# wangrui2025/GDKVM

Hardware: AMD Instinct MI355X
Metric: frames/sec (GDKVM forward + argmax mask), EchoNet 112x112x32 clips (higher is better)
Workload: dtype bf16; 1 GPU; BASELINE.json configs[1]: EchoNet-Dynamic 112x112x32 bf16 inference, batch=16 per GPU; clips_per_gpu=16, frames_per_clip=32, image=112x112, heads=1, key_dim=64, rule=delta_sequential, world_size=1, ranks_seen=1

## Files before the change

gdkvm_amd/csrc/conv3x3_tile.hip:

```cpp
#include <atomic>
#include "gdkvm_device.hpp"

namespace {

constexpr int CT_CK = 64;
constexpr int CT_PIX = 160;
constexpr int CT_SLOTS = CT_PIX / 16;
constexpr int CT_MAXMT = 13;
constexpr int CT_VARIANT_128 = 4, CT_VARIANT_64 = 3;

struct ConvTileArgs {
    const bf16_t* x; const bf16_t* w; const float* bias; const bf16_t* res; bf16_t* y;
    const bf16_t* x2; int C1;
    int N, H, W, C, K;
    int fpt, th, tiles_y, ntiles;
    int bw, bh, band_px, npieces;
    int relu;
    float inv_band, inv_bw, inv_tw, inv_w;
    int perm;
};
struct ConvUpArgs : ConvTileArgs {
    int hl, wl, nlr;
    int stage_px, nstage;
    int stage_off;
    int nrp;
    float inv_slr, inv_wl, inv_ncp, inv_nrp;
};

__host__ __device__ __forceinline__ int ct_channel(int kt, int j, int perm)
{
    return perm ? 32 * (kt >> 1) + 8 * (j >> 2) + 4 * (kt & 1) + (j & 3) : 16 * kt + j;
}

template <int NWN, int NTW, bool PK, int NWV = 8, int MAXMT = CT_MAXMT, bool UP = false>
__global__ __launch_bounds__(64 * NWV, (NWV == 4 ? 2 : 1)) void conv3x3_tile_kernel(std::conditional_t<UP, ConvUpArgs, ConvTileArgs> a)
{
    constexpr int MW = NWV / NWN, MTW = (MAXMT + MW - 1) / MW;
    extern __shared__ __attribute__((aligned(16))) unsigned char ct_band[];
    const int tid = threadIdx.x, lane = tid & 63, li = lane & 15, g = lane >> 4;
    const int w = __builtin_amdgcn_readfirstlane(tid >> 6), wn = w % NWN, wm = w / NWN;
    const int H = a.H, W = a.W, C = a.C, K = a.K, BW = a.bw;
    const int band_bytes = a.npieces * 1024, nchunk = C / CT_CK;
    const int tpix = a.fpt * a.th * W;
    const int co0 = blockIdx.y * (16 * NTW * NWN) + 16 * NTW * wn;

    f32x4 bias4[NTW];
#pragma unroll
    for (int nt = 0; nt < NTW; ++nt) {
        const int kt = min(co0 / 16 + nt, K / 16 - 1);
        const float* bp = a.bias + ct_channel(kt, 4 * g, a.perm);
        asm volatile("global_load_dwordx4 %0, %1, off" : "=&v"(bias4[nt]) : "v"(bp) : "memory");
    }

    constexpr int PP = NWV == 8 ? 7 : 8;
    const int cs1 = a.C1, cs2 = a.x2 ? C - a.C1 : C;
    unsigned g_off1[PP], g_off2[PP];
#pragma unroll
    for (int u = 0; u < PP; ++u) {
        const int j = w + NWV * u, d = 64 * j + lane, pix = d / CT_SLOTS, c = d - CT_SLOTS * pix;
        const int f = idx_div(pix, a.inv_band), r = pix - f * (a.bh * BW), by = idx_div(r, a.inv_bw), bx = r - by * BW;
        const int sp = (f * H + by - 1) * W + bx - 1;
        const bool live = j < a.npieces && c < 8 && pix < a.band_px && bx >= 1 && bx <= W && (a.tiles_y > 1 || (by >= 1 && by <= a.th));
        g_off1[u] = live ? (unsigned)(sp * cs1 * 2 + c * 16) : RSRC_DEAD;
        g_off2[u] = live ? (unsigned)(sp * cs2 * 2 + c * 16) : RSRC_DEAD;
        if constexpr (UP) {
            const int spx = d >> 3, c8 = d & 7;
            const int sf = idx_div(spx, a.inv_slr), sr = spx - sf * (a.nlr * a.wl), lr = idx_div(sr, a.inv_wl), lx = sr - lr * a.wl;
            g_off1[u] = j < a.nstage && spx < a.stage_px ? (unsigned)((((sf * a.hl + lr) * a.wl + lx) * cs1 + c8 * 8) * 2) : RSRC_DEAD;
        }
    }
    const unsigned lds0 = (unsigned)reinterpret_cast<uintptr_t>(ct_band);
    const int nlive = max(0, (a.npieces - w + NWV - 1) / NWV);
    int nlive_up = 0, stage_off = 0;
    if constexpr (UP) { nlive_up = max(0, (a.nstage - w + NWV - 1) / NWV); stage_off = a.stage_off; }
    struct Geo { int px0, npx, row0, r0, lr0, nfr; };
    auto geo_of = [&](int tile) __attribute__((always_inline)) {
        const int ty = tile % a.tiles_y, fg = tile / a.tiles_y;
        Geo q;
        q.px0 = fg * a.fpt * H * W;
        q.npx = min(a.fpt, a.N - fg * a.fpt) * H * W;
        q.row0 = ty * a.th * W;
        q.r0 = q.lr0 = q.nfr = 0;
        if constexpr (UP) {
            q.r0 = ty * a.th; q.lr0 = max((q.r0 - 2) >> 1, 0); q.nfr = min(a.fpt, a.N - fg * a.fpt);
        }
        return q;
    };
    auto fetch = [&](const Geo q, int chunk, int buf) __attribute__((always_inline)) {
        const bool second = a.x2 != nullptr && chunk * CT_CK >= a.C1;
        const int cs = second ? cs2 : cs1;
        const bool up = UP && !second;
        const bf16_t* base = (second ? a.x2 : a.x) + (long long)(up ? q.px0 >> 2 : q.px0) * cs;
        const __amdgpu_buffer_rsrc_t rsrc = make_rsrc(base, (up ? q.npx >> 2 : q.npx) * cs * 2);
        unsigned ts = (unsigned)((q.row0 * cs + chunk * CT_CK - (second ? a.C1 : 0)) * 2);
        unsigned dst0 = lds0 + buf * band_bytes + 1024 * w;
        int nl = nlive;
        if constexpr (UP) {
            ts = up ? (unsigned)((q.lr0 * (W >> 1) * cs + chunk * CT_CK) * 2) : ts;
            dst0 = up ? lds0 + stage_off + 1024 * w : dst0;
            nl = up ? nlive_up : nlive;
        }
#pragma unroll
        for (int u = 0; u < PP; ++u) {
            const unsigned dst = u < nl ? dst0 + 1024 * NWV * u : lds0 + 2 * band_bytes;
            unsigned go;
            if constexpr (UP) go = g_off1[u] ^ ((g_off1[u] ^ g_off2[u]) & (second ? ~0u : 0u));
            else go = second ? g_off2[u] : g_off1[u];
            __builtin_amdgcn_raw_ptr_buffer_load_lds(rsrc, lds_dma_dst(dst), 16, (int)(go + ts), 0, 0, 0);
        }
    };

    int tile = blockIdx.x;
    Geo cur = geo_of(min(tile, a.ntiles - 1));
    if (tile < a.ntiles) fetch(cur, 0, 0);

    unsigned pbase[MTW];
#pragma unroll
    for (int m = 0; m < MTW; ++m) {
        const int p = min(16 * (wm + MW * m) + li, tpix - 1);
        const int f = idx_div(p, a.inv_tw), r = p - f * (a.th * W), py = idx_div(r, a.inv_w), px = r - py * W;
        pbase[m] = (unsigned)(((f * a.bh + py) * BW + px) * CT_PIX + g * 16);
    }
    const bf16_t* wrow[NTW];
#pragma unroll
    for (int nt = 0; nt < NTW; ++nt) {
        const int kt = min(co0 / 16 + nt, K / 16 - 1);
        if constexpr (PK) wrow[nt] = a.w + (size_t)kt * (9 * C * 16) + lane * 8;
        else wrow[nt] = a.w + (size_t)ct_channel(kt, li, a.perm) * 9 * C + 8 * g;
    }

    const int nks = nchunk * 18;
    static_assert(NTW == 1 || NTW == 2, "wwait names the fragments of one or two output tiles");
    struct WF { bf16x8 f[NTW]; };
    auto wload = [&](WF& o, int ks) __attribute__((always_inline)) {
        ks = ks >= nks ? ks - nks : ks;
        size_t off;
        if constexpr (PK) off = (size_t)ks * 512;
        else {
            const int chunk = ks / 18, r = ks - 18 * chunk, tap = r >> 1, kh = r & 1;
            off = (size_t)tap * C + chunk * CT_CK + 32 * kh;
        }
#pragma unroll
        for (int nt = 0; nt < NTW; ++nt) asm volatile("global_load_dwordx4 %0, %1, off" : "=&v"(o.f[nt]) : "v"(wrow[nt] + off) : "memory");
    };
    auto wwait = [&](WF& o, auto nc) __attribute__((always_inline)) {
        constexpr int N = decltype(nc)::value;
        if constexpr (NTW == 1) asm volatile("s_waitcnt vmcnt(%1)" : "+v"(o.f[0]) : "n"(N) : "memory");
        else asm volatile("s_waitcnt vmcnt(%2)" : "+v"(o.f[0]), "+v"(o.f[1]) : "n"(N) : "memory");
    };
    int gc = 0;
    constexpr int WD = 3, KU = 6;
    WF wr[WD];
#pragma unroll
    for (int j = 0; j < WD; ++j) wload(wr[j], j);
    for (; tile < a.ntiles; tile += gridDim.x) {
        const Geo nxt = geo_of(min(tile + (int)gridDim.x, a.ntiles - 1));
        f32x4 acc[MTW][NTW];
#pragma unroll
        for (int m = 0; m < MTW; ++m)
#pragma unroll
            for (int nt = 0; nt < NTW; ++nt) acc[m][nt] = f32x4{0.f, 0.f, 0.f, 0.f};
        for (int chunk = 0; chunk < nchunk; ++chunk, ++gc) {
            const int buf = gc & 1;
            asm volatile("s_waitcnt vmcnt(%0) lgkmcnt(0)" ::"n"(WD * NTW) : "memory");
            asm volatile("s_barrier" ::: "memory");
            if constexpr (UP) if (chunk * CT_CK < a.C1) {
                const unsigned stg = lds0 + stage_off;
                unsigned char* const bandw = ct_band + buf * band_bytes;
                const int hl = H >> 1, wl = W >> 1, ncp = wl + 1, ip0 = (cur.r0 - 2) >> 1;
                const int nitems = a.fpt * a.nrp * ncp * 8;
#pragma unroll 1
                for (int i = tid; i < nitems; i += 64 * NWV) {
                    const int c8 = i & 7, t = i >> 3;
                    const int t2 = idx_div(t, a.inv_ncp), jp = t - t2 * ncp - 1, f = idx_div(t2, a.inv_nrp), ip = ip0 + t2 - f * a.nrp;
                    const int y0 = 2 * ip + 1, x0o = 2 * jp + 1;
                    const int by0 = y0 - cur.r0 + 1;
                    const bool vy[2] = {y0 >= 0 && y0 < H, y0 + 1 >= 0 && y0 + 1 < H}, vx[2] = {x0o >= 0, x0o + 1 < W};
                    u32x4 o[2][2] = {};
                    if ((vy[0] || vy[1]) && f < cur.nfr) {
                        const int ra = max(ip, 0) - cur.lr0, rb = min(ip + 1, hl - 1) - cur.lr0;
                        const int xa_ = max(jp, 0), xb_ = min(jp + 1, wl - 1);
                        const unsigned s0 = stg + (f * a.nlr + ra) * wl * 128 + c8 * 16, s1 = stg + (f * a.nlr + rb) * wl * 128 + c8 * 16;
                        u32x4 t00, t01, t10, t11;
                        asm volatile("ds_read_b128 %0, %1" : "=&v"(t00) : "v"(s0 + xa_ * 128) : "memory");
                        asm volatile("ds_read_b128 %0, %1" : "=&v"(t01) : "v"(s0 + xb_ * 128) : "memory");
                        asm volatile("ds_read_b128 %0, %1" : "=&v"(t10) : "v"(s1 + xa_ * 128) : "memory");
                        asm volatile("ds_read_b128 %0, %1" : "=&v"(t11) : "v"(s1 + xb_ * 128) : "memory");
                        asm volatile("s_waitcnt lgkmcnt(0)" : "+v"(t00), "+v"(t01), "+v"(t10), "+v"(t11) :: "memory");
                        const float ly[2] = {0.25f, y0 + 1 == 0 ? 0.f : 0.75f}, hy[2] = {0.75f, 1.f - ly[1]};
                        bilerp2x_bf16x8(t00, t01, t10, t11, hy, ly, o);
                    }
#pragma unroll
                    for (int ey = 0; ey < 2; ++ey) {
                        if (by0 + ey < 0 || by0 + ey >= a.bh) continue;
                        const bool rowin = vy[ey] && f < cur.nfr;
#pragma unroll
                        for (int e = 0; e < 2; ++e) {
                            const u32x4 z = {0u, 0u, 0u, 0u};
                            *reinterpret_cast<u32x4*>(bandw + ((f * a.bh + by0 + ey) * BW + x0o + 1 + e) * CT_PIX + c8 * 16) = rowin && vx[e] ? o[ey][e] : z;
                        }
                    }
                }
                asm volatile("s_waitcnt lgkmcnt(0)" ::: "memory");
                asm volatile("s_barrier" ::: "memory");
            }
            {
                const bool more = chunk + 1 < nchunk;
                Geo q;
                q.px0 = more ? cur.px0 : nxt.px0; q.npx = more ? cur.npx : nxt.npx; q.row0 = more ? cur.row0 : nxt.row0;
                q.r0 = q.lr0 = q.nfr = 0;
                if constexpr (UP) q.lr0 = more ? cur.lr0 : nxt.lr0;
                fetch(q, more ? chunk + 1 : 0, buf ^ 1);
            }
            const unsigned char* band = ct_band + buf * band_bytes;
            auto load_x = [&](bf16x8 (&xb)[MTW], int r) __attribute__((always_inline)) {
                r = min(r, 17);
                const int tap = r >> 1, kh = r & 1, dy = tap / 3, dx = tap - 3 * dy;
                const unsigned off = (unsigned)((dy * BW + dx) * CT_PIX + kh * 64);
#pragma unroll
                for (int m = 0; m < MTW; ++m) {
                    xb[m] = *reinterpret_cast<const bf16x8*>(band + pbase[m] + off);
                }
            };
            auto mfmas = [&](const bf16x8 (&xb)[MTW], const WF& wfr) __attribute__((always_inline)) {
#pragma unroll
                for (int m = 0; m < MTW; ++m)
#pragma unroll
                    for (int nt = 0; nt < NTW; ++nt) {
                        acc[m][nt] = __builtin_amdgcn_mfma_f32_16x16x32_bf16(wfr.f[nt], xb[m], acc[m][nt], 0, 0, 0);
                    }
            };
            const int ksb = chunk * 18;
            bf16x8 xa[MTW], xb[MTW];
            load_x(xa, 0);
            auto trip = [&](int r0, auto firstc) __attribute__((always_inline)) {
                constexpr bool FIRST = decltype(firstc)::value;
                static_for<0, KU>([&](auto jc) {
                    constexpr int j = decltype(jc)::value;
                    wwait(wr[j % WD], std::integral_constant<int, (WD - 1) * NTW + (FIRST && j < WD ? PP : 0)>{});
                    if constexpr (j % 2 == 0) { load_x(xb, r0 + j + 1); mfmas(xa, wr[j % WD]); }
                    else { load_x(xa, r0 + j + 1); mfmas(xb, wr[j % WD]); }
                    wload(wr[j % WD], ksb + r0 + j + WD);
                    __builtin_amdgcn_sched_barrier(0);
                });
            };
            trip(0, std::true_type{});
#pragma unroll 1
            for (int r0 = KU; r0 < 18; r0 += KU) trip(r0, std::false_type{});
        }
        {
            const int ty = tile % a.tiles_y, fg = tile / a.tiles_y;
            const float lo = a.relu ? 0.f : -INFINITY;
            if (NTW == 2 && a.perm) {
                if (co0 < K) {
                    unsigned o[MTW];
#pragma unroll
                    for (int m = 0; m < MTW; ++m) {
                        const int p = 16 * (wm + MW * m) + li;
                        const int pc = min(p, tpix - 1);
                        const int f = idx_div(pc, a.inv_tw), r = pc - f * (a.th * W), py = idx_div(r, a.inv_w), px = r - py * W;
                        const int n = fg * a.fpt + f, yy = ty * a.th + py;
                        o[m] = p < tpix && n < a.N && yy < H ? (unsigned)(((n * H + yy) * W + px) * K + co0 + 8 * g) : ~0u;
                    }
                    bf16_t* const yout = a.y;
                    const bf16_t* const resp = a.res;
                    const unsigned ofallback = (unsigned)(co0 + 8 * g);
                    auto finish = [&](auto resc) __attribute__((always_inline)) {
                        constexpr bool RES = decltype(resc)::value;
                        static_for<0, (MTW + 3) / 4>([&](auto bc) {
                            constexpr int M0 = 4 * decltype(bc)::value, M1 = M0 + 4 < MTW ? M0 + 4 : MTW;
                            u32x4 rr[4] = {};
                            if constexpr (RES) {
#pragma unroll
                                for (int m = M0; m < M1; ++m)
                                {
                                    const bf16_t* const rp = resp + (o[m] != ~0u ? o[m] : ofallback);
                                    asm volatile("global_load_dwordx4 %0, %1, off" : "=&v"(rr[m - M0]) : "v"(rp) : "memory");
                                }
                                asm volatile("s_waitcnt vmcnt(0)" : "+v"(rr[0]), "+v"(rr[1]), "+v"(rr[2]), "+v"(rr[3]) :: "memory");
                            }
#pragma unroll
                            for (int m = M0; m < M1; ++m) {
                                f32x2 v[4];
#pragma unroll
                                for (int q = 0; q < 4; ++q)
                                    v[q] = f32x2{acc[m][q >> 1][2 * (q & 1)], acc[m][q >> 1][2 * (q & 1) + 1]} + f32x2{bias4[q >> 1][2 * (q & 1)], bias4[q >> 1][2 * (q & 1) + 1]};
                                if constexpr (RES) {
#pragma unroll
                                    for (int q = 0; q < 4; ++q) v[q] += unpack_bf16x2(rr[m - M0][q]);
                                }
                                u32x4 ow;
#pragma unroll
                                for (int q = 0; q < 4; ++q) {
                                    v[q] = __builtin_elementwise_max(v[q], f32x2{lo, lo});
                                    ow[q] = pack_bf16x2(v[q][0], v[q][1]);
                                }
                                bf16_t* const yp = yout + o[m];
                                if (o[m] != ~0u) asm volatile("global_store_dwordx4 %0, %1, off\n\ts_nop 1" :: "v"(yp), "v"(ow) : "memory");
                            }
                        });
                    };
                    if (a.res) finish(std::true_type{}); else finish(std::false_type{});
                }
            } else {
#pragma unroll
                for (int m = 0; m < MTW; ++m) {
                    const int p = 16 * (wm + MW * m) + li;
                    if (p >= tpix) continue;
                    const int f = idx_div(p, a.inv_tw), r = p - f * (a.th * W), py = idx_div(r, a.inv_w), px = r - py * W;
                    const int n = fg * a.fpt + f, yy = ty * a.th + py;
                    if (n >= a.N || yy >= H) continue;
                    const size_t opix = (((size_t)n * H + yy) * W + px) * K;
#pragma unroll
                    for (int nt = 0; nt < NTW; ++nt) {
                        if (co0 + 16 * nt >= K) continue;
                        const size_t o = opix + ct_channel(co0 / 16 + nt, 4 * g, a.perm);
                        f32x4 v = acc[m][nt] + bias4[nt];
                        if (a.res) v += unpack_bf16x4(*reinterpret_cast<const uint2*>(a.res + o));
                        v = __builtin_elementwise_max(v, f32x4{lo, lo, lo, lo});
                        *reinterpret_cast<uint2*>(a.y + o) = pack_bf16x4(v);
                    }
                }
            }
        }
        cur = nxt;
    }
    asm volatile("s_waitcnt vmcnt(0)" ::: "memory");
}

__global__ __launch_bounds__(256) void conv3x3_pack_kernel(const uint4* w, uint4* packed, int K, int C)
{
    const int nks = C / CT_CK * 18;
    const size_t total = (size_t)(K / 16) * nks * 64;
    for (size_t i = (size_t)blockIdx.x * 256 + threadIdx.x; i < total; i += (size_t)gridDim.x * 256) {
        const int lane = (int)(i & 63), li = lane & 15, g = lane >> 4;
        const size_t f = i >> 6;
        const int ks = (int)(f % nks), kt = (int)(f / nks);
        const int chunk = ks / 18, r = ks - 18 * chunk, tap = r >> 1, kh = r & 1;
        packed[i] = w[(((size_t)ct_channel(kt, li, K % 32 == 0) * 9 + tap) * C + chunk * CT_CK + 32 * kh + 8 * g) / 8];
    }
}

__global__ __launch_bounds__(256) void conv3x3_pack_dgrad_kernel(const bf16_t* w, uint4* packed, int K, int C)
{
    const int nks = K / CT_CK * 18;
    const size_t total = (size_t)(C / 16) * nks * 64;
    for (size_t i = (size_t)blockIdx.x * 256 + threadIdx.x; i < total; i += (size_t)gridDim.x * 256) {
        const int lane = (int)(i & 63), li = lane & 15, g = lane >> 4;
        const size_t f = i >> 6;
        const int ks = (int)(f % nks), ct = (int)(f / nks);
        const int chunk = ks / 18, r = ks - 18 * chunk, tap = r >> 1, kh = r & 1;
        const int c = ct_channel(ct, li, C % 32 == 0), ftap = 8 - tap;
        const bf16_t* src = w + ((size_t)(chunk * CT_CK + 32 * kh + 8 * g) * 9 + ftap) * C + c;
        unsigned short e[8];
#pragma unroll
        for (int j = 0; j < 8; ++j) e[j] = src[(size_t)j * 9 * C];
        packed[i] = make_uint4(e[0] | (unsigned)e[1] << 16, e[2] | (unsigned)e[3] << 16, e[4] | (unsigned)e[5] << 16, e[6] | (unsigned)e[7] << 16);
    }
}

}

struct PackTrainLayer { const float* w; uint4* fwd; uint4* dgrad; int K, C; long long sK, sC, sR, sS; };
struct PackTrainArgs { PackTrainLayer l[GDKVM_PACK_MAX_LAYERS]; };

namespace {
__global__ __launch_bounds__(256) void conv3x3_pack_train_kernel(PackTrainArgs a)
{
    const PackTrainLayer L = a.l[blockIdx.y];
    if (!L.w) return;
    const int K = L.K, C = L.C;
    const size_t nf = (size_t)(K / 16) * (C / CT_CK * 18) * 64, nd = (size_t)(C / 16) * (K / CT_CK * 18) * 64;
    for (size_t i = (size_t)blockIdx.x * 256 + threadIdx.x; i < nf + nd; i += (size_t)gridDim.x * 256) {
        const bool fwd = i < nf;
        const size_t ii = fwd ? i : i - nf;
        const int lane = (int)(ii & 63), li = lane & 15, g = lane >> 4;
        const size_t f = ii >> 6;
        float e[8];
        if (fwd) {
            const int nks = C / CT_CK * 18, ks = (int)(f % nks), kt = (int)(f / nks);
            const int chunk = ks / 18, r = ks - 18 * chunk, tap = r >> 1, kh = r & 1;
            const float* src = L.w + (long long)ct_channel(kt, li, K % 32 == 0) * L.sK + (long long)(tap / 3) * L.sR + (long long)(tap % 3) * L.sS
                               + (long long)(chunk * CT_CK + 32 * kh + 8 * g) * L.sC;
#pragma unroll
            for (int j = 0; j < 8; ++j) e[j] = src[(long long)j * L.sC];
        } else {
            const int nks = K / CT_CK * 18, ks = (int)(f % nks), ct = (int)(f / nks);
            const int chunk = ks / 18, r = ks - 18 * chunk, tap = r >> 1, kh = r & 1, ftap = 8 - tap;
            const float* src = L.w + (long long)ct_channel(ct, li, C % 32 == 0) * L.sC + (long long)(ftap / 3) * L.sR + (long long)(ftap % 3) * L.sS
                               + (long long)(chunk * CT_CK + 32 * kh + 8 * g) * L.sK;
#pragma unroll
            for (int j = 0; j < 8; ++j) e[j] = src[(long long)j * L.sK];
        }
        const uint4 o = pack_bf16x8(e);
        (fwd ? L.fwd : L.dgrad)[ii] = o;
    }
}
}

extern "C" int gdkvm_conv3x3_pack_weights_train(int nlayers, const void* const* w, void* const* packed_fwd, void* const* packed_dgrad,
                                                const int* K, const int* C, const long long* strides, void* stream)
{
    if (nlayers < 0 || nlayers > GDKVM_PACK_MAX_LAYERS) return gdkvm_fail(GDKVM_ERR_SHAPE, "conv3x3_pack_weights_train: %d layers (at most %d per call)", nlayers, GDKVM_PACK_MAX_LAYERS);
    if (nlayers == 0) return GDKVM_OK;
    if (!w || !packed_fwd || !packed_dgrad || !K || !C || !strides) return gdkvm_fail(GDKVM_ERR_ARG, "conv3x3_pack_weights_train: null pointer");
    PackTrainArgs a{};
    for (int i = 0; i < nlayers; ++i) {
        if (K[i] <= 0 || C[i] <= 0 || K[i] % CT_CK || C[i] % CT_CK)
            return gdkvm_fail(GDKVM_ERR_SHAPE, "conv3x3_pack_weights_train: layer %d K=%d C=%d (multiples of 64)", i, K[i], C[i]);
        if (!w[i] || !packed_fwd[i] || !packed_dgrad[i] || !gdkvm_aligned16(packed_fwd[i]) || !gdkvm_aligned16(packed_dgrad[i]))
            return gdkvm_fail(GDKVM_ERR_ARG, "conv3x3_pack_weights_train: layer %d: null or unaligned pointer", i);
        a.l[i] = PackTrainLayer{static_cast<const float*>(w[i]), static_cast<uint4*>(packed_fwd[i]), static_cast<uint4*>(packed_dgrad[i]), K[i], C[i],
                                strides[4 * i], strides[4 * i + 1], strides[4 * i + 2], strides[4 * i + 3]};
    }
    if (int rc = gdkvm_check_device()) return rc;
    hipLaunchKernelGGL(conv3x3_pack_train_kernel, dim3(48, (unsigned)nlayers), dim3(256), 0, static_cast<hipStream_t>(stream), a);
    GDKVM_LAUNCH_CHECK("conv3x3_pack_train_kernel");
    return GDKVM_OK;
}

extern "C" int gdkvm_conv3x3_pack_weights_dgrad(const void* w, void* packed, int K, int C, int io_dtype, void* stream)
{
    if (io_dtype != GDKVM_BF16) return gdkvm_fail(GDKVM_ERR_DTYPE, "conv3x3_pack_weights_dgrad: only bf16 is implemented");
    if (K <= 0 || C <= 0 || K % CT_CK || C % 16) return gdkvm_fail(GDKVM_ERR_SHAPE, "conv3x3_pack_weights_dgrad: K=%d C=%d (K a multiple of 64, C of 16)", K, C);
    if (!w || !packed || !gdkvm_aligned16(w) || !gdkvm_aligned16(packed)) return gdkvm_fail(GDKVM_ERR_ARG, "conv3x3_pack_weights_dgrad: null or unaligned pointer");
    if (int rc = gdkvm_check_device()) return rc;
    const size_t total = (size_t)(C / 16) * (K / CT_CK * 18) * 64;
    hipLaunchKernelGGL(conv3x3_pack_dgrad_kernel, dim3((unsigned)((total + 255) / 256)), dim3(256), 0, static_cast<hipStream_t>(stream),
                       static_cast<const bf16_t*>(w), static_cast<uint4*>(packed), K, C);
    GDKVM_LAUNCH_CHECK("conv3x3_pack_dgrad_kernel");
    return GDKVM_OK;
}

extern "C" int gdkvm_conv3x3_pack_weights(const void* w, void* packed, int K, int C, int io_dtype, void* stream)
{
    if (io_dtype != GDKVM_BF16) return gdkvm_fail(GDKVM_ERR_DTYPE, "conv3x3_pack_weights: only bf16 is implemented");
    if (K <= 0 || C <= 0 || K % 16 || C % CT_CK) return gdkvm_fail(GDKVM_ERR_SHAPE, "conv3x3_pack_weights: K=%d C=%d (K a multiple of 16, C of 64)", K, C);
    if (!w || !packed || !gdkvm_aligned16(w) || !gdkvm_aligned16(packed)) return gdkvm_fail(GDKVM_ERR_ARG, "conv3x3_pack_weights: null or unaligned pointer");
    if (int rc = gdkvm_check_device()) return rc;
    const size_t total = (size_t)(K / 16) * (C / CT_CK * 18) * 64;
    hipLaunchKernelGGL(conv3x3_pack_kernel, dim3((unsigned)((total + 255) / 256)), dim3(256), 0, static_cast<hipStream_t>(stream),
                       static_cast<const uint4*>(w), static_cast<uint4*>(packed), K, C);
    GDKVM_LAUNCH_CHECK("conv3x3_pack_kernel");
    return GDKVM_OK;
}

namespace {
template <int NWN, int NTW, int NWV = 8, int MAXMT = CT_MAXMT>
void launch_tile(bool packed, dim3 grid, size_t lds, hipStream_t st, const ConvTileArgs& a)
{
    if (packed) hipLaunchKernelGGL((conv3x3_tile_kernel<NWN, NTW, true, NWV, MAXMT>), grid, dim3(64 * NWV), lds, st, a);
    else hipLaunchKernelGGL((conv3x3_tile_kernel<NWN, NTW, false, NWV, MAXMT>), grid, dim3(64 * NWV), lds, st, a);
}
template <int NWN, int NTW, int NWV = 8, int MAXMT = CT_MAXMT>
bool setattr_tile()
{
    return hipFuncSetAttribute(reinterpret_cast<const void*>(conv3x3_tile_kernel<NWN, NTW, true, NWV, MAXMT>), hipFuncAttributeMaxDynamicSharedMemorySize, 113 * 1024) == hipSuccess
        && hipFuncSetAttribute(reinterpret_cast<const void*>(conv3x3_tile_kernel<NWN, NTW, false, NWV, MAXMT>), hipFuncAttributeMaxDynamicSharedMemorySize, 113 * 1024) == hipSuccess;
}
constexpr size_t CT_UP_LDS = 80 * 1024;
template <int NWN, int NTW>
bool setattr_up()
{
    return hipFuncSetAttribute(reinterpret_cast<const void*>(conv3x3_tile_kernel<NWN, NTW, true, 4, 7, true>), hipFuncAttributeMaxDynamicSharedMemorySize, (int)CT_UP_LDS) == hipSuccess;
}

bool tile_geometry(ConvTileArgs& a, int maxpix, int maxpieces)
{
    const int N = a.N, H = a.H, W = a.W;
    if (H * W <= maxpix) { a.th = H; a.fpt = maxpix / (H * W); a.tiles_y = 1; if (a.fpt > N) a.fpt = N; }
    else { a.fpt = 1; a.th = maxpix / W; if (a.th < 1) return false; a.tiles_y = (H + a.th - 1) / a.th; }
    a.bw = W + 2; a.bh = a.th + 2;
    auto pieces = [&]() { a.band_px = a.fpt * a.bh * a.bw; return (a.band_px * CT_SLOTS + 63) / 64; };
    while (pieces() > maxpieces && a.fpt > 1) --a.fpt;
    while (pieces() > maxpieces && a.th > 1) { --a.th; a.bh = a.th + 2; a.tiles_y = (H + a.th - 1) / a.th; }
    a.npieces = pieces();
    if (a.npieces > maxpieces) return false;
    a.inv_band = 1.0f / (float)(a.bh * a.bw); a.inv_bw = 1.0f / (float)a.bw;
    a.inv_tw = 1.0f / (float)(a.th * W); a.inv_w = 1.0f / (float)W;
    const long long groups = (N + a.fpt - 1) / a.fpt;
    const long long ntiles = groups * a.tiles_y;
    if (ntiles <= 0 || ntiles > 0x7fffffffLL) return false;
    a.ntiles = (int)ntiles;
    return true;
}
}

int gdkvm_conv3x3_upcat_launch(const void* lo, const void* x2, int C1, const void* w, const float* bias, const void* residual, void* y,
                               int N, int C, int H, int W, int K, int relu, hipStream_t st)
{
    if (C % CT_CK || K % 16 || W > 64 || W < 2 || H < 2 || (H | W) & 1 || N < 1 || !x2 || C1 <= 0 || C1 >= C || C1 % CT_CK) return 1;
    ConvUpArgs a;
    a.x2 = static_cast<const bf16_t*>(x2); a.C1 = C1;
    a.x = static_cast<const bf16_t*>(lo); a.w = static_cast<const bf16_t*>(w); a.bias = bias;
    a.res = static_cast<const bf16_t*>(residual); a.y = static_cast<bf16_t*>(y);
    a.N = N; a.H = H; a.W = W; a.C = C; a.K = K; a.relu = relu;
    if (!tile_geometry(a, 16 * 7, 32)) return 1;
    if ((long long)(a.fpt * H + 2) * W * (C1 > C - C1 ? C1 : C - C1) * 2 >= 0x7fffffffLL) return 1;
    a.perm = K % 32 == 0;
    a.hl = H / 2; a.wl = W / 2;
    a.nlr = a.bh / 2 + 2 < a.hl ? a.bh / 2 + 2 : a.hl;
    a.stage_px = a.fpt * a.nlr * a.wl;
    a.nstage = (a.stage_px + 7) / 8;
    if (a.nstage > 32) return 1;
    a.inv_slr = 1.0f / (float)(a.nlr * a.wl); a.inv_wl = 1.0f / (float)a.wl;
    a.nrp = a.bh / 2 + 1; a.inv_ncp = 1.0f / (float)(a.wl + 1); a.inv_nrp = 1.0f / (float)a.nrp;
    a.stage_off = 2 * a.npieces * 1024 + 1024;
    const size_t lds = (size_t)a.stage_off + (size_t)a.nstage * 1024;
    if (lds > CT_UP_LDS) return 1;
    const int kwg = K % 128 == 0 ? 128 : 64;
    const int gy = (K + kwg - 1) / kwg;
    int per = 512 / gy; if (per < 1) per = 1;
    const int gx = a.ntiles < per ? a.ntiles : per;
    static std::atomic<unsigned long long> done_mask{0};
    int dev = 0;
    if (hipGetDevice(&dev) != hipSuccess) return 1;
    const unsigned long long bit = 1ull << (dev & 63);
    if (!(done_mask.load(std::memory_order_relaxed) & bit)) {
        if (!setattr_up<4, 2>() || !setattr_up<2, 2>()) return 1;
        done_mask.fetch_or(bit, std::memory_order_relaxed);
    }
    if (kwg == 128) hipLaunchKernelGGL((conv3x3_tile_kernel<4, 2, true, 4, 7, true>), dim3(gx, gy), dim3(256), lds, st, a);
    else hipLaunchKernelGGL((conv3x3_tile_kernel<2, 2, true, 4, 7, true>), dim3(gx, gy), dim3(256), lds, st, a);
    return 0;
}

int gdkvm_conv3x3_tile_launch(const void* x, const void* x2, int C1, const void* w, const float* bias, const void* residual, void* y,
                              int N, int C, int H, int W, int K, int relu, int variant, int packed, hipStream_t st)
{
    if (variant == 0 && K % 128 == 0 && CT_VARIANT_128 == 4) {
        if (gdkvm_conv3x3_tile_launch(x, x2, C1, w, bias, residual, y, N, C, H, W, K, relu, 4, packed, st) == 0) return 0;
        variant = 2;
    }
    if (variant == 0 && K % 128 != 0 && (H * W <= 16 * 7 || 2 * W <= 16 * 7)) {
        if (gdkvm_conv3x3_tile_launch(x, x2, C1, w, bias, residual, y, N, C, H, W, K, relu, 5, packed, st) == 0) return 0;
        variant = 3;
    }
    if (C % CT_CK || K % 16 || W > 64 || W < 1 || H < 1 || N < 1 || variant < 0 || variant > 5) return 1;
    if (variant == 4 && K % 128) return 1;
    const bool half = variant == 4 || variant == 5;
    if (x2 && (C1 <= 0 || C1 >= C || C1 % CT_CK)) return 1;
    ConvTileArgs a;
    a.x2 = static_cast<const bf16_t*>(x2); a.C1 = x2 ? C1 : C;
    a.x = static_cast<const bf16_t*>(x); a.w = static_cast<const bf16_t*>(w); a.bias = bias;
    a.res = static_cast<const bf16_t*>(residual); a.y = static_cast<bf16_t*>(y);
    a.N = N; a.H = H; a.W = W; a.C = C; a.K = K; a.relu = relu;
    const int maxpix = half ? 16 * 7 : 16 * CT_MAXMT;
    const int maxpieces = half ? 32 : 56;
    if (!tile_geometry(a, maxpix, maxpieces)) return 1;
    if ((long long)(a.fpt * H + 2) * W * (x2 ? (C1 > C - C1 ? C1 : C - C1) : C) * 2 >= 0x7fffffffLL) return 1;
    a.perm = K % 32 == 0;
    const long long ntiles = a.ntiles;
    if (variant == 0) variant = K % 128 == 0 ? 2 : CT_VARIANT_64;
    const int kwg = (variant == 2 || variant == 4) ? 128 : 64;
    const int gy = (K + kwg - 1) / kwg;
    const size_t lds = (size_t)2 * a.npieces * 1024 + 1024;
    int per = (half ? 512 : 256) / gy; if (per < 1) per = 1;
    const int gx = (int)(ntiles < per ? ntiles : per);
    static std::atomic<unsigned long long> done_mask{0};
    int dev = 0;
    if (hipGetDevice(&dev) != hipSuccess) return 1;
    const unsigned long long bit = 1ull << (dev & 63);
    if (!(done_mask.load(std::memory_order_relaxed) & bit)) {
        if (!setattr_tile<4, 1>() || !setattr_tile<4, 2>() || !setattr_tile<2, 2>() || !setattr_tile<4, 2, 4, 7>() || !setattr_tile<2, 2, 4, 7>()) return 1;
        done_mask.fetch_or(bit, std::memory_order_relaxed);
    }
    switch (variant) {
        case 1: launch_tile<4, 1>(packed, dim3(gx, gy), lds, st, a); break;
        case 2: launch_tile<4, 2>(packed, dim3(gx, gy), lds, st, a); break;
        case 4: launch_tile<4, 2, 4, 7>(packed, dim3(gx, gy), lds, st, a); break;
        case 5: launch_tile<2, 2, 4, 7>(packed, dim3(gx, gy), lds, st, a); break;
        default: launch_tile<2, 2>(packed, dim3(gx, gy), lds, st, a); break;
    }
    return 0;
}
```

Baseline: 668,800 frames/s.

## Stack frames contiguously into conv3x3 tiles to eliminate padded-tile waste

Adds a stacked tiling mode for the half-size (4-wave) conv3x3 variants. Tiles now span frame boundaries so that each tile of maxpix pixels is fully used, instead of padding when H*W or H does not divide the tile size. The band gains extra halo rows for frame crossings, and row-liveness masks prevent reading across frame edges. The persistent grid size is rounded to a multiple of the phase count. This adds index arithmetic and a larger band in exchange for fewer idle MFMA rows.

```diff
diff --git a/gdkvm_amd/csrc/conv3x3_tile.hip b/gdkvm_amd/csrc/conv3x3_tile.hip
--- a/gdkvm_amd/csrc/conv3x3_tile.hip
+++ b/gdkvm_amd/csrc/conv3x3_tile.hip
@@ -18,6 +18,8 @@
     int relu;
     float inv_band, inv_bw, inv_tw, inv_w;
     int perm;
+    int stk, sg;
+    float inv_hw, inv_h1;
 };
 struct ConvUpArgs : ConvTileArgs {
     int hl, wl, nlr;
@@ -43,6 +45,11 @@
     const int band_bytes = a.npieces * 1024, nchunk = C / CT_CK;
     const int tpix = a.fpt * a.th * W;
     const int co0 = blockIdx.y * (16 * NTW * NWN) + 16 * NTW * wn;
+    const bool stk = NWV == 4 && !UP && a.stk != 0;
+    const int ph = stk ? (int)(blockIdx.x % (unsigned)a.stk) : 0, s0 = ph * a.th, f0 = stk ? s0 / H : 0, m0 = s0 - f0 * H;
+    const int poff = stk ? ph * tpix : 0, pper = stk ? H * W : a.th * W, rmul = stk ? H + 1 : a.bh, rsub = stk ? s0 + f0 : 0;
+    const float inv_pper = stk ? a.inv_hw : a.inv_tw;
+    const int tdiv = stk ? a.stk : a.tiles_y, fpg = stk ? a.sg : a.fpt;
 
     f32x4 bias4[NTW];
 #pragma unroll
@@ -59,8 +66,11 @@
     for (int u = 0; u < PP; ++u) {
         const int j = w + NWV * u, d = 64 * j + lane, pix = d / CT_SLOTS, c = d - CT_SLOTS * pix;
         const int f = idx_div(pix, a.inv_band), r = pix - f * (a.bh * BW), by = idx_div(r, a.inv_bw), bx = r - by * BW;
-        const int sp = (f * H + by - 1) * W + bx - 1;
-        const bool live = j < a.npieces && c < 8 && pix < a.band_px && bx >= 1 && bx <= W && (a.tiles_y > 1 || (by >= 1 && by <= a.th));
+        const int uu = by - 1 + m0, k = idx_div(max(uu, 0), a.inv_h1), rr = uu - k * (H + 1), srow = s0 - m0 + k * H + rr;
+        const bool srow_live = uu >= 0 && rr < H && (srow < s0 + a.th || (srow == s0 + a.th && rr != 0));
+        const int sp = ((stk ? srow : f * H + by - 1)) * W + bx - 1;
+        const bool row_live = stk ? srow_live : a.tiles_y > 1 || (by >= 1 && by <= a.th);
+        const bool live = j < a.npieces && c < 8 && pix < a.band_px && bx >= 1 && bx <= W && row_live;
         g_off1[u] = live ? (unsigned)(sp * cs1 * 2 + c * 16) : RSRC_DEAD;
         g_off2[u] = live ? (unsigned)(sp * cs2 * 2 + c * 16) : RSRC_DEAD;
         if constexpr (UP) {
@@ -75,11 +85,11 @@
     if constexpr (UP) { nlive_up = max(0, (a.nstage - w + NWV - 1) / NWV); stage_off = a.stage_off; }
     struct Geo { int px0, npx, row0, r0, lr0, nfr; };
     auto geo_of = [&](int tile) __attribute__((always_inline)) {
-        const int ty = tile % a.tiles_y, fg = tile / a.tiles_y;
+        const int ty = tile % tdiv, fg = tile / tdiv;
         Geo q;
-        q.px0 = fg * a.fpt * H * W;
-        q.npx = min(a.fpt, a.N - fg * a.fpt) * H * W;
-        q.row0 = ty * a.th * W;
+        q.px0 = fg * fpg * H * W;
+        q.npx = min(fpg, a.N - fg * fpg) * H * W;
+        q.row0 = stk ? 0 : ty * a.th * W;
         q.r0 = q.lr0 = q.nfr = 0;
         if constexpr (UP) {
             q.r0 = ty * a.th; q.lr0 = max((q.r0 - 2) >> 1, 0); q.nfr = min(a.fpt, a.N - fg * a.fpt);
@@ -117,9 +127,9 @@
     unsigned pbase[MTW];
 #pragma unroll
     for (int m = 0; m < MTW; ++m) {
-        const int p = min(16 * (wm + MW * m) + li, tpix - 1);
-        const int f = idx_div(p, a.inv_tw), r = p - f * (a.th * W), py = idx_div(r, a.inv_w), px = r - py * W;
-        pbase[m] = (unsigned)(((f * a.bh + py) * BW + px) * CT_PIX + g * 16);
+        const int p = poff + min(16 * (wm + MW * m) + li, tpix - 1);
+        const int f = idx_div(p, inv_pper), r = p - f * pper, py = idx_div(r, a.inv_w), px = r - py * W;
+        pbase[m] = (unsigned)(((f * rmul + py - rsub) * BW + px) * CT_PIX + g * 16);
     }
     const bf16_t* wrow[NTW];
 #pragma unroll
@@ -249,7 +259,7 @@
             for (int r0 = KU; r0 < 18; r0 += KU) trip(r0, std::false_type{});
         }
         {
-            const int ty = tile % a.tiles_y, fg = tile / a.tiles_y;
+            const int fg = tile / tdiv, y0 = stk ? 0 : (tile - fg * tdiv) * a.th, n0 = fg * fpg;
             const float lo = a.relu ? 0.f : -INFINITY;
             if (NTW == 2 && a.perm) {
                 if (co0 < K) {
@@ -257,9 +267,9 @@
 #pragma unroll
                     for (int m = 0; m < MTW; ++m) {
                         const int p = 16 * (wm + MW * m) + li;
-                        const int pc = min(p, tpix - 1);
-                        const int f = idx_div(pc, a.inv_tw), r = pc - f * (a.th * W), py = idx_div(r, a.inv_w), px = r - py * W;
-                        const int n = fg * a.fpt + f, yy = ty * a.th + py;
+                        const int pc = poff + min(p, tpix - 1);
+                        const int f = idx_div(pc, inv_pper), r = pc - f * pper, py = idx_div(r, a.inv_w), px = r - py * W;
+                        const int n = n0 + f, yy = y0 + py;
                         o[m] = p < tpix && n < a.N && yy < H ? (unsigned)(((n * H + yy) * W + px) * K + co0 + 8 * g) : ~0u;
                     }
                     bf16_t* const yout = a.y;
@@ -307,8 +317,9 @@
                 for (int m = 0; m < MTW; ++m) {
                     const int p = 16 * (wm + MW * m) + li;
                     if (p >= tpix) continue;
-                    const int f = idx_div(p, a.inv_tw), r = p - f * (a.th * W), py = idx_div(r, a.inv_w), px = r - py * W;
-                    const int n = fg * a.fpt + f, yy = ty * a.th + py;
+                    const int pc = poff + p;
+                    const int f = idx_div(pc, inv_pper), r = pc - f * pper, py = idx_div(r, a.inv_w), px = r - py * W;
+                    const int n = n0 + f, yy = y0 + py;
                     if (n >= a.N || yy >= H) continue;
                     const size_t opix = (((size_t)n * H + yy) * W + px) * K;
 #pragma unroll
@@ -465,9 +476,33 @@
     return hipFuncSetAttribute(reinterpret_cast<const void*>(conv3x3_tile_kernel<NWN, NTW, true, 4, 7, true>), hipFuncAttributeMaxDynamicSharedMemorySize, (int)CT_UP_LDS) == hipSuccess;
 }
 
+bool stacked_geometry(ConvTileArgs& a, int maxpix, int maxpieces, int maxgrid)
+{
+    const int N = a.N, H = a.H, W = a.W, hw = H * W;
+    int gcd = hw, b = maxpix;
+    while (b) { const int t = gcd % b; gcd = b; b = t; }
+    a.stk = hw / gcd; a.sg = maxpix / gcd;
+    if (a.stk > maxgrid) return false;
+    a.fpt = 1; a.tiles_y = 1; a.th = maxpix / W; a.bw = W + 2;
+    int cross = 0;
+    for (int ph = 0; ph < a.stk; ++ph) { const int s0 = ph * a.th, c = (s0 + a.th - 1) / H - s0 / H; if (c > cross) cross = c; }
+    a.bh = a.th + 2 + cross;
+    a.band_px = a.bh * a.bw;
+    a.npieces = (a.band_px * CT_SLOTS + 63) / 64;
+    if (a.npieces > maxpieces) return false;
+    a.inv_band = 1.0f / (float)(a.bh * a.bw); a.inv_bw = 1.0f / (float)a.bw;
+    a.inv_tw = 1.0f / (float)(a.th * W); a.inv_w = 1.0f / (float)W;
+    a.inv_hw = 1.0f / (float)hw; a.inv_h1 = 1.0f / (float)(H + 1);
+    const long long ntiles = (long long)(N / a.sg) * a.stk + ((long long)(N % a.sg) * H + a.th - 1) / a.th;
+    if (ntiles <= 0 || ntiles > 0x7fffffffLL) return false;
+    a.ntiles = (int)ntiles;
+    return true;
+}
+
 bool tile_geometry(ConvTileArgs& a, int maxpix, int maxpieces)
 {
     const int N = a.N, H = a.H, W = a.W;
+    a.stk = 0; a.sg = 0; a.inv_hw = a.inv_h1 = 0.f;
     if (H * W <= maxpix) { a.th = H; a.fpt = maxpix / (H * W); a.tiles_y = 1; if (a.fpt > N) a.fpt = N; }
     else { a.fpt = 1; a.th = maxpix / W; if (a.th < 1) return false; a.tiles_y = (H + a.th - 1) / a.th; }
     a.bw = W + 2; a.bh = a.th + 2;
@@ -547,15 +582,17 @@
     a.N = N; a.H = H; a.W = W; a.C = C; a.K = K; a.relu = relu;
     const int maxpix = half ? 16 * 7 : 16 * CT_MAXMT;
     const int maxpieces = half ? 32 : 56;
-    if (!tile_geometry(a, maxpix, maxpieces)) return 1;
-    if ((long long)(a.fpt * H + 2) * W * (x2 ? (C1 > C - C1 ? C1 : C - C1) : C) * 2 >= 0x7fffffffLL) return 1;
-    a.perm = K % 32 == 0;
-    const long long ntiles = a.ntiles;
     if (variant == 0) variant = K % 128 == 0 ? 2 : CT_VARIANT_64;
     const int kwg = (variant == 2 || variant == 4) ? 128 : 64;
     const int gy = (K + kwg - 1) / kwg;
+    int per = (half ? 512 : 256) / gy; if (per < 1) per = 1;
+    const bool padded = H * W <= maxpix ? maxpix % (H * W) != 0 : H % (maxpix / W) != 0;
+    if (!(half && maxpix % W == 0 && padded && stacked_geometry(a, maxpix, maxpieces, per)) && !tile_geometry(a, maxpix, maxpieces)) return 1;
+    if ((long long)((a.stk ? a.sg : a.fpt) * H + 2) * W * (x2 ? (C1 > C - C1 ? C1 : C - C1) : C) * 2 >= 0x7fffffffLL) return 1;
+    a.perm = K % 32 == 0;
+    const long long ntiles = a.ntiles;
     const size_t lds = (size_t)2 * a.npieces * 1024 + 1024;
-    int per = (half ? 512 : 256) / gy; if (per < 1) per = 1;
+    if (a.stk) per -= per % a.stk;
     const int gx = (int)(ntiles < per ? ntiles : per);
     static std::atomic<unsigned long long> done_mask{0};
     int dev = 0;
```

Result: faster. 681,800 frames/s (median of 6 runs) (+1.9%).
